# EricSteinberger/PokerRL

Measured on NVIDIA H100. Metric: CFR+ iterations/s, higher is better.
Workload: dtype f32

## Files before the change

pokerrl_b200/csrc/cfr_board.cu:

```cuda
#include <cuda_runtime.h>
#include <stdint.h>
#include <type_traits>

#include "pokerrl_b200.h"
#include "prl_common.cuh"

namespace {

constexpr int kDeck = 52;
constexpr int kBoardCards = 5;
constexpr int kLiveCards = kDeck - kBoardCards;
constexpr int kLive = kLiveCards * (kLiveCards - 1) / 2;
constexpr int kLdb = 1088;
constexpr int kRowLen = kLiveCards - 1;
constexpr int kRowPad = 48;
constexpr int kRowSeg = 12;
constexpr int kErStride = kLiveCards;
constexpr int kZeroSlot = kLive + 1;
constexpr int kRange = 1326;

constexpr int kRecBytes = kLdb * 8;
constexpr int kShBytes = kLdb * 2;
constexpr int kRowIdxBytes = kLiveCards * kRowPad * 2;
constexpr int kBlobA = kRecBytes + kShBytes;
constexpr int kBlobBytes = kBlobA + kRowIdxBytes;
static_assert(kBlobA % 16 == 0 && kRowIdxBytes % 16 == 0, "bulk copies move multiples of 16 bytes");

#ifndef PRL_BV_RED
#define PRL_BV_RED 1
#endif
#ifndef PRL_BV_P1PIPE
#define PRL_BV_P1PIPE 1
#endif
#ifndef PRL_BV_FOLDLIN
#define PRL_BV_FOLDLIN 1
#endif
#ifndef PRL_BV_ERT
#define PRL_BV_ERT 1
#endif
#ifndef PRL_BV_ROWTOTF
#define PRL_BV_ROWTOTF 1
#endif
#ifndef PRL_BV_NEWTON
#define PRL_BV_NEWTON 1
#endif
#ifndef PRL_BV_PF
#define PRL_BV_PF 1
#endif
#ifndef PRL_BV_STAMPS
#define PRL_BV_STAMPS 0
#endif
constexpr int kVP1Pipe = PRL_BV_P1PIPE;
constexpr bool kVRed = PRL_BV_RED, kVFoldLin = PRL_BV_FOLDLIN, kVErT = PRL_BV_ERT;

constexpr int kThreads = 384;
constexpr int kPerThread = 3;
constexpr int kWarps = kThreads / 32;

struct Nodes15 {
    int v[15];
};
constexpr unsigned long long pack_nodes(Nodes15 t) {
    unsigned long long r = 0;
    for (int i = 0; i < 15; ++i) r |= (unsigned long long)(t.v[i] + 1) << (4 * i);
    return r;
}
constexpr int unpack_node(unsigned long long t, int i) { return (int)((t >> (4 * i)) & 0xF) - 1; }

template <class SH>
struct ShapeOps {
    static constexpr int kind(int i) { return unpack_node(SH::kKind, i); }
    static constexpr int parent(int i) { return unpack_node(SH::kParent, i); }
    static constexpr int first_child(int i) { return unpack_node(SH::kFirstChild, i); }
    static constexpr int n_children(int i) { return unpack_node(SH::kNChildren, i); }
    static constexpr int vec_index(int i) {
        int n = 0;
        for (int k = 0; k < i; ++k) n += (kind(k) == kind(i));
        return n;
    }
// ... 28 lines not shown

struct ShapeFHP : ShapeOps<ShapeFHP> {
    static constexpr int N = 15;
    static constexpr unsigned long long kKind = pack_nodes({{1, 0, 0, 4, 1, 3, 4, 1, 3, 4, 0, 3, 4, 3, 4}});
    static constexpr unsigned long long kParent = pack_nodes({{-1, 0, 0, 1, 1, 2, 2, 2, 4, 4, 4, 7, 7, 10, 10}});
    static constexpr unsigned long long kFirstChild = pack_nodes({{1, 3, 5, -1, 8, -1, -1, 11, -1, -1, 13, -1, -1, -1, -1}});
    static constexpr unsigned long long kNChildren = pack_nodes({{2, 2, 3, 0, 3, 0, 0, 2, 0, 0, 2, 0, 0, 0, 0}});
    static constexpr int n_sd = 5, n_fold = 4;
    static constexpr int rows = 14;
    static constexpr int fold_coef(int P, int f, int v) {
        constexpr int c[2][4][5] = {{{0, 1, 0, 0, 0}, {1, 0, -1, 0, -1}, {0, 1, 0, -1, 0}, {0, 0, 0, 0, 1}},
                                    {{1, -1, 1, -1, 0}, {0, 0, 1, 0, 0}, {0, 0, 0, 1, 0}, {0, 0, 1, 0, -1}}};
        return c[P][f][v];
    }
};

struct ShapeFHPShort : ShapeOps<ShapeFHPShort> {
    static constexpr int N = 9;
    static constexpr unsigned long long kKind = pack_nodes({{1, 0, 0, 4, 1, 3, 4, 3, 4}});
    static constexpr unsigned long long kParent = pack_nodes({{-1, 0, 0, 1, 1, 2, 2, 4, 4}});
    static constexpr unsigned long long kFirstChild = pack_nodes({{1, 3, 5, -1, 7, -1, -1, -1, -1}});
    static constexpr unsigned long long kNChildren = pack_nodes({{2, 2, 2, 0, 2, 0, 0, 0, 0}});
    static constexpr int n_sd = 3, n_fold = 2;
    static constexpr int rows = 8;
    static constexpr int fold_coef(int P, int f, int v) {
        constexpr int c[2][2][3] = {{{0, 1, 0}, {1, 0, -1}}, {{1, -1, 1}, {0, 0, 1}}};
        return c[P][f][v];
    }
};

template <class SH>
constexpr bool shape_consistent() {
    return SH::count(4) == SH::n_sd && SH::count(3) == SH::n_fold && SH::rows_of_seat(0) + SH::rows_of_seat(1) == SH::rows &&
           SH::N <= 15 && SH::n_fold % 2 == 0;
}
static_assert(shape_consistent<ShapeFHP>() && shape_consistent<ShapeFHPShort>(), "shape");

template <int I, int N, class F>
__device__ __forceinline__ void static_for(F&& f) {
    if constexpr (I < N) {
        f(std::integral_constant<int, I>{});
        static_for<I + 1, N>(f);
    }
}
template <int I, int N, class F>
__device__ __forceinline__ void static_for_down(F&& f) {
    if constexpr (I < N) {
        f(std::integral_constant<int, N - 1>{});
        static_for_down<I, N - 1>(f);
    }
}

constexpr int kErVec = kLiveCards * kErStride;
template <class SH>
struct SweepSmem {
    static constexpr int kNVec = SH::n_sd + SH::n_fold;
    static constexpr int kSOff = 0;
    static constexpr int kErOff = kSOff + kNVec * kLdb * 4;
    static constexpr int kErBytes = ((SH::n_sd * kErVec * 4) + 15) & ~15;
    static constexpr int kBlobOff = kErOff + kErBytes;
    static constexpr int kRowIdxOff = kBlobOff + 2 * kBlobA;
    static constexpr int kCsOff = kRowIdxOff + kRowIdxBytes;
    static constexpr int kCsdOff = kCsOff + SH::n_fold * kRowPad * 4;
    static constexpr int kMiscOff = kCsdOff + SH::n_fold * kRowPad * 8;
    static constexpr int kMiscBytes = (SH::n_sd * 16 + SH::n_sd * 16) * 8 + 8 * 4;
    static constexpr int kRowTotOff = kMiscOff + kMiscBytes;
    static constexpr int kRowTotBytes = SH::n_sd * kRowPad * 8;
    static constexpr int kBarOff = kRowTotOff + kRowTotBytes;
    static constexpr int kSmemBytes = kBarOff + 32;
    static_assert(kBlobOff % 16 == 0 && kRowIdxOff % 16 == 0 && kCsdOff % 8 == 0 && kMiscOff % 8 == 0 && kRowTotOff % 8 == 0 &&
                      kBarOff % 8 == 0, "alignment");
    static_assert(2 * (kSmemBytes + 1024) <= 233472, "two CTAs per SM (228 KB of shared memory per H100 SM)");
    static_assert(SH::n_fold <= 8, "tf[8]");
};

struct SweepArgs {
    prl_board_game_t g;
    const float* trunk_reach_opp;
    int iter, delay;
    float m_old, m_new;
    int pair;
    float m_old_due, m_new_due;
    int src_own, src_opp;
    float rw;
    float defer_w;
    double fx_scale;
    float sc[16];
};

__device__ __forceinline__ uint32_t smem_u32(const void* p) { return (uint32_t)__cvta_generic_to_shared(p); }
__device__ __forceinline__ void mbar_init(uint64_t* bar, int count) {
    asm volatile("mbarrier.init.shared::cta.b64 [%0], %1;" ::"r"(smem_u32(bar)), "r"(count) : "memory");
}
__device__ __forceinline__ void mbar_expect_tx(uint64_t* bar, uint32_t bytes) {
    asm volatile("mbarrier.arrive.expect_tx.shared::cta.b64 _, [%0], %1;" ::"r"(smem_u32(bar)), "r"(bytes) : "memory");
}
__device__ __forceinline__ void bulk_g2s(void* dst, const void* src, uint32_t bytes, uint64_t* bar) {
    asm volatile("cp.async.bulk.shared::cluster.global.mbarrier::complete_tx::bytes [%0], [%1], %2, [%3];" ::"r"(smem_u32(dst)),
                 "l"(src), "r"(bytes), "r"(smem_u32(bar))
                 : "memory");
}
__device__ __forceinline__ void bulk_prefetch_l2(const void* src, uint32_t bytes) {
    asm volatile("cp.async.bulk.prefetch.L2.global [%0], %1;" ::"l"(src), "r"(bytes) : "memory");
}
__device__ __forceinline__ void mbar_wait(uint64_t* bar, uint32_t parity) {
    uint32_t ok;
    do {
        asm volatile(
            "{\n\t.reg .pred p;\n\tmbarrier.try_wait.parity.shared::cta.b64 p, [%1], %2;\n\tselp.u32 %0, 1, 0, p;\n\t}"
            : "=r"(ok)
            : "r"(smem_u32(bar)), "r"(parity)
            : "memory");
    } while (!ok);
}
__device__ __forceinline__ void fence_async_shared() { asm volatile("fence.proxy.async.shared::cta;" ::: "memory"); }

#if PRL_BV_STAMPS
constexpr int kStampCtas = 512, kStampUnits = 16, kStampEvery = 32, kStampSlots = 8;
__device__ long long g_stamps[kStampCtas * kStampUnits * kStampSlots];
#endif
__device__ __forceinline__ void stamp(int it, int slot) {
#if PRL_BV_STAMPS
    if (threadIdx.x == 0 && blockIdx.x < kStampCtas && it % kStampEvery == 0 && it / kStampEvery < kStampUnits) {
        long long* r = g_stamps + ((size_t)blockIdx.x * kStampUnits + it / kStampEvery) * kStampSlots;
        r[slot] = clock64();
        if (slot == 0) {
            unsigned smid;
            asm volatile("mov.u32 %0, %%smid;" : "=r"(smid));
            r[6] = smid;
            r[7] = it;
        }
    }
#endif
}

template <int A>
__device__ __forceinline__ void node_strategy(const float (&g)[A], int src, float (&s)[A]) {
    if (src == 1) {
#pragma unroll
        for (int a = 0; a < A; ++a) s[a] = g[a];
        return;
    }
    float sum = 0.0f;
#pragma unroll
    for (int a = 0; a < A; ++a) {
        s[a] = fmaxf(g[a], 0.0f);
        sum += s[a];
    }
    const bool pos = sum > 0.0f;
    const float sm = fmaxf(sum, 1e-37f);
    float inv;
    asm("rcp.approx.ftz.f32 %0, %1;" : "=f"(inv) : "f"(sm));
    if (PRL_BV_NEWTON) inv = fmaf(inv, fmaf(-sm, inv, 1.0f), inv);
    inv = pos ? inv : 0.0f;
    const float uni = pos ? 0.0f : 1.0f / (float)A;
#pragma unroll
    for (int a = 0; a < A; ++a) s[a] = fmaf(s[a], inv, uni);
}

__device__ __forceinline__ float avg_step(float m_old, float avg, float m_new, float s) {
    return __fmaf_rn(m_old, avg, __fmul_rn(m_new, s));
}

__device__ __forceinline__ float ld_stream(const float* p) { return __ldcs(p); }
__device__ __forceinline__ void st_stream(float* p, float v) { __stcs(p, v); }

template <class SH, int P, bool EVAL, bool DEFER = false, bool P1ONLY = false, bool AVG = true>
__global__ void __launch_bounds__(kThreads, 2) board_sweep_kernel(const SweepArgs a) {
    static_assert(!(EVAL && DEFER) && (!P1ONLY || DEFER) && (AVG || (!EVAL && !DEFER)), "variants");
    using M = SweepSmem<SH>;
    constexpr int NSD = SH::n_sd, NF = SH::n_fold;
    extern __shared__ __align__(128) unsigned char smem[];
    float* S = reinterpret_cast<float*>(smem + M::kSOff);
    float* Er = reinterpret_cast<float*>(smem + M::kErOff);
    float* cs = reinterpret_cast<float*>(smem + M::kCsOff);
    double* csd = reinterpret_cast<double*>(smem + M::kCsdOff);
    double* wsum = reinterpret_cast<double*>(smem + M::kMiscOff);
    double* wexc = wsum + NSD * 16;
    float* tf = reinterpret_cast<float*>(wexc + NSD * 16);
    uint64_t* bars = reinterpret_cast<uint64_t*>(smem + M::kBarOff);
    const int16_t* rowidx = reinterpret_cast<const int16_t*>(smem + M::kRowIdxOff);
    double* rowtot = reinterpret_cast<double*>(smem + M::kRowTotOff);
    constexpr bool kLin = kVFoldLin && !EVAL;

    const int tid = threadIdx.x, lane = tid & 31, warp = tid >> 5;
    const prl_board_game_t& G = a.g;
    const int nb = G.n_boards;
    constexpr int OPP = 1 - P;
    constexpr int ROWS = SH::rows;
    constexpr int OWN0 = (P == 0) ? 0 : SH::rows_of_seat(0);
    constexpr int OPP0 = (P == 0) ? SH::rows_of_seat(0) : 0;
    constexpr int NOWN = SH::rows_of_seat(P), NOPP = SH::rows_of_seat(OPP);
    constexpr size_t kBoardFloats = (size_t)ROWS * kLdb;
    const unsigned char* blob_g = reinterpret_cast<const unsigned char*>(G.tables);
    const float* tab_opp = (EVAL && a.src_opp >= 1) ? G.avg : G.regret;
    const float* tab_own = (EVAL && a.src_own >= 1) ? G.avg : G.regret;
    const int asis_opp = (EVAL && a.src_opp == 1) ? 1 : 0, asis_own = (EVAL && a.src_own == 1) ? 1 : 0;
    const bool do_avg = !EVAL && !DEFER && AVG && a.iter >= a.delay;
    const bool pair = do_avg && a.pair;
    const bool defer_now = DEFER && a.defer_w != 0.0f;
    const bool read_avg = do_avg && (pair ? a.m_old_due : a.m_old) != 0.0f;

    long long* wp = reinterpret_cast<long long*>(G.w_private) + (size_t)blockIdx.x * 2 * kRange;
    for (int h = tid; h < 2 * kRange; h += kThreads) wp[h] = 0;
    for (int v = 0; v < M::kNVec; ++v)
        for (int i = kLive + tid; i < kLdb; i += kThreads) S[v * kLdb + i] = 0.0f;
    if (tid == 0) {
        mbar_init(&bars[0], 1);
        mbar_init(&bars[1], 1);
        mbar_init(&bars[2], 1);
        fence_async_shared();
    }
    __syncthreads();
    int j = blockIdx.x;
    auto prefetch_rows = [&](int jj) {
        bulk_prefetch_l2(tab_opp + (size_t)jj * kBoardFloats + (size_t)OPP0 * kLdb, NOPP * kLdb * 4);
        bulk_prefetch_l2(tab_own + (size_t)jj * kBoardFloats + (size_t)OWN0 * kLdb, NOWN * kLdb * 4);
        if (read_avg) bulk_prefetch_l2(G.avg + (size_t)jj * kBoardFloats + (size_t)OWN0 * kLdb, NOWN * kLdb * 4);
        if (defer_now) bulk_prefetch_l2(G.avg + (size_t)jj * kBoardFloats + (size_t)OPP0 * kLdb, NOPP * kLdb * 4);
    };
    constexpr bool kPfPhase = PRL_BV_PF && !EVAL;
    auto prefetch_opp = [&](int jj) {
        bulk_prefetch_l2(tab_opp + (size_t)jj * kBoardFloats + (size_t)OPP0 * kLdb, NOPP * kLdb * 4);
        if (defer_now) bulk_prefetch_l2(G.avg + (size_t)jj * kBoardFloats + (size_t)OPP0 * kLdb, NOPP * kLdb * 4);
    };
    auto prefetch_own = [&](int jj) {
        bulk_prefetch_l2(tab_own + (size_t)jj * kBoardFloats + (size_t)OWN0 * kLdb, NOWN * kLdb * 4);
        if (read_avg) bulk_prefetch_l2(G.avg + (size_t)jj * kBoardFloats + (size_t)OWN0 * kLdb, NOWN * kLdb * 4);
    };
    if (tid == 0 && j < nb) {
        mbar_expect_tx(&bars[0], kBlobA);
        bulk_g2s(smem + M::kBlobOff, blob_g + (size_t)j * kBlobBytes, kBlobA, &bars[0]);
        if (!P1ONLY) {
            mbar_expect_tx(&bars[2], kRowIdxBytes);
            bulk_g2s(smem + M::kRowIdxOff, blob_g + (size_t)j * kBlobBytes + kBlobA, kRowIdxBytes, &bars[2]);
        }
        if constexpr (kPfPhase) prefetch_opp(j);
        else prefetch_rows(j);
    }

    constexpr int kP1Ahead = kVP1Pipe ? kVP1Pipe : kPerThread;
    float p1_g[kP1Ahead][NOPP], p1_x0[kP1Ahead];
    auto p1_load_k = [&](int jj, const int16_t* sh_jj, int k, float (&g)[NOPP], float& x0) {
        const int i = min(tid + k * kThreads, kLive - 1);
        const float* rows = tab_opp + (size_t)jj * kBoardFloats + (size_t)OPP0 * kLdb + i;
#pragma unroll
        for (int r = 0; r < NOPP; ++r) g[r] = ld_stream(rows + (size_t)r * kLdb);
        x0 = __ldg(a.trunk_reach_opp + sh_jj[i]);
    };
    auto p1_load = [&](int jj, const int16_t* sh_jj) {
#pragma unroll
        for (int k = 0; k < kP1Ahead; ++k) p1_load_k(jj, sh_jj, k, p1_g[k], p1_x0[k]);
    };

    for (int it = 0; j < nb; j += gridDim.x, ++it) {
        const int buf = it & 1;
        const unsigned char* blob = smem + M::kBlobOff + buf * kBlobA;
        const uint64_t* rec = reinterpret_cast<const uint64_t*>(blob);
        const int16_t* sh = reinterpret_cast<const int16_t*>(blob + kRecBytes);
        const int jn = j + gridDim.x;
        stamp(it, 0);
        if (tid == 0 && jn < nb) {
            mbar_expect_tx(&bars[buf ^ 1], kBlobA);
            bulk_g2s(smem + M::kBlobOff + (buf ^ 1) * kBlobA, blob_g + (size_t)jn * kBlobBytes, kBlobA, &bars[buf ^ 1]);
            if constexpr (!kPfPhase) prefetch_rows(jn);
        }
        const float prob = __ldg(G.board_prob + j);
        if (it == 0) {
            mbar_wait(&bars[buf], 0);
            p1_load(j, sh);
        }

        auto p1_hand = [&](int k, const float (&gk)[NOPP], float x0k) {
            const int i = tid + k * kThreads;
            if (i < kLive) {
                float x[SH::N];
                x[0] = x0k * prob;
                static_for<0, SH::N>([&](auto I) {
                    constexpr int n = decltype(I)::value;
                    constexpr int A = SH::n_children(n);
                    if constexpr (SH::kind(n) <= 1) {
                        constexpr int fc = SH::first_child(n);
                        if constexpr (SH::kind(n) == OPP) {
                            constexpr int r0 = SH::row_of(fc);
                            float gg[A], s[A];
#pragma unroll
                            for (int c = 0; c < A; ++c) gg[c] = gk[r0 - OPP0 + c];
                            node_strategy<A>(gg, asis_opp, s);
#pragma unroll
                            for (int c = 0; c < A; ++c) x[fc + c] = x[n] * s[c];
                            if constexpr (DEFER) {
                                if (defer_now) {
                                    float* arow = G.avg + (size_t)j * kBoardFloats + i;
#pragma unroll
                                    for (int c = 0; c < A; ++c) {
                                        float* ap = arow + (size_t)(r0 + c) * kLdb;
                                        st_stream(ap, __fadd_rn(ld_stream(ap), __fmul_rn(x[fc + c], a.defer_w)));
                                    }
                                }
                            }
                        } else {
#pragma unroll
                            for (int c = 0; c < A; ++c) x[fc + c] = x[n];
                        }
                    } else if constexpr (SH::kind(n) == 4) {
                        S[SH::vec_index(n) * kLdb + i] = x[n];
                    } else {
                        S[(NSD + SH::vec_index(n)) * kLdb + i] = x[n];
                    }
                });
            }
        };
        if constexpr (kVP1Pipe == 1) {
            float gB[NOPP], gC[NOPP], xB = 0.0f, xC = 0.0f;
            p1_load_k(j, sh, 1, gB, xB);
            p1_hand(0, p1_g[0], p1_x0[0]);
            p1_load_k(j, sh, 2, gC, xC);
            p1_hand(1, gB, xB);
            p1_hand(2, gC, xC);
        } else {
#pragma unroll
            for (int k = 0; k < kPerThread; ++k) p1_hand(k, p1_g[k], p1_x0[k]);
        }
        __syncthreads();
        stamp(it, 1);
        if (kPfPhase && tid == 0) {
            if constexpr (P1ONLY) {
                if (jn < nb) prefetch_opp(jn);
            } else {
                prefetch_own(j);
            }
        }
        if constexpr (!P1ONLY) {

        mbar_wait(&bars[2], it & 1);
        float a0[NSD], a1[NSD], a2[NSD];
        double pre[NSD];
        constexpr int kQuadThreads = kLiveCards * 4;
        constexpr int kSdSplit = (NSD + 1) / 2, kFoldSplit = NF / 2;
        if (warp < (2 * kQuadThreads + 31) / 32) {
            const int grp = (tid >= kQuadThreads) ? 1 : 0;
            const int t = tid - grp * kQuadThreads;
            const bool row_live = t < kQuadThreads;
            const int lc = row_live ? (t >> 2) : (kLiveCards - 1), q = tid & 3;
            const unsigned qmask = 0xFu << (lane & 28);
            const uint2* rp = reinterpret_cast<const uint2*>(rowidx + lc * kRowPad + q * kRowSeg);
            const uint2 w0 = rp[0], w1 = rp[1], w2 = rp[2];
            const unsigned pk[6] = {w0.x, w0.y, w1.x, w1.y, w2.x, w2.y};
            int idx[kRowSeg];
#pragma unroll
            for (int e = 0; e < kRowSeg; ++e) idx[e] = (pk[e >> 1] >> ((e & 1) * 16)) & 0xffffu;
            const int v_lo = grp ? kSdSplit : 0, v_hi = grp ? NSD : kSdSplit;
#pragma unroll 1
            for (int v = v_lo; v < v_hi; ++v) {
                const float* Sv = S + v * kLdb;
                float inc[kRowSeg];
                float run = 0.0f;
                double drun = 0.0;
#pragma unroll
                for (int e = 0; e < kRowSeg; ++e) {
                    const float xv = Sv[idx[e]];
                    inc[e] = run;
                    run += xv;
                    if constexpr (kLin && !PRL_BV_ROWTOTF) drun += (double)xv;
                }
                if constexpr (kLin) {
                    if constexpr (PRL_BV_ROWTOTF) drun = (double)run;
                    drun += __shfl_xor_sync(qmask, drun, 1, 4);
                    drun += __shfl_xor_sync(qmask, drun, 2, 4);
                    if (row_live && q == 0) rowtot[v * kRowPad + lc] = drun;
                }
                float sc = run;
                float tt = __shfl_up_sync(qmask, sc, 1, 4);
                if (q >= 1) sc += tt;
                tt = __shfl_up_sync(qmask, sc, 2, 4);
                if (q >= 2) sc += tt;
                const float half = 0.5f * __shfl_sync(qmask, sc, 3, 4);
                const float off = (sc - run) - half;
                float* row = Er + v * kErVec + (kVErT ? q * kRowSeg * kErStride + lc : lc * kErStride + q * kRowSeg);
#pragma unroll
                for (int e = 0; e < kRowSeg; ++e)
                    if (row_live && q * kRowSeg + e < kErStride) row[kVErT ? e * kErStride : e] = off + inc[e];
            }
#pragma unroll 1
            for (int f = kFoldSplit * grp; f < (kLin ? 0 : kFoldSplit * grp + kFoldSplit); ++f) {
                const float* Sv = S + (NSD + f) * kLdb;
                double run = 0.0;
#pragma unroll
                for (int e = 0; e < kRowSeg; ++e) run += (double)Sv[idx[e]];
                run += __shfl_xor_sync(qmask, run, 1, 4);
                run += __shfl_xor_sync(qmask, run, 2, 4);
                if (row_live && q == 0) csd[f * kRowPad + lc] = run;
            }
        }
        __syncwarp();
        {
            const int b0 = 3 * tid;
#pragma unroll
            for (int v = 0; v < NSD; ++v) {
                const float* Sv = S + v * kLdb;
                a0[v] = (b0 < kLive) ? Sv[b0] : 0.0f;
                a1[v] = (b0 + 1 < kLive) ? Sv[b0 + 1] : 0.0f;
                a2[v] = (b0 + 2 < kLive) ? Sv[b0 + 2] : 0.0f;
                const double loc = ((double)a0[v] + (double)a1[v]) + (double)a2[v];
                double incw = loc;
#pragma unroll
                for (int o = 1; o < 32; o <<= 1) {
                    const double tt = __shfl_up_sync(0xffffffffu, incw, o);
                    if (lane >= o) incw += tt;
                }
                pre[v] = incw - loc;
                if (lane == 31) wsum[v * 16 + warp] = incw;
            }
        }
        const float mult = __ldg(G.board_mult + j);
        const double fx = (double)mult * a.fx_scale;
        const float* own_rows = tab_own + (size_t)j * kBoardFloats + (size_t)OWN0 * kLdb;
        float* reg_rows = G.regret + (size_t)j * kBoardFloats + (size_t)OWN0 * kLdb;
        float* avg_rows = G.avg + (size_t)j * kBoardFloats + (size_t)OWN0 * kLdb;
        auto p3_pos = [&](int k) -> int { return tid + k * kThreads; };
        float gA[NOWN], aA[NOWN], gB[NOWN], aB[NOWN];
        auto p3_load = [&](int k, float (&g)[NOWN], float (&av)[NOWN]) {
            const int i = min(p3_pos(k), kLive - 1);
#pragma unroll
            for (int r = 0; r < NOWN; ++r) g[r] = ld_stream(own_rows + (size_t)r * kLdb + i);
#pragma unroll
            for (int r = 0; r < NOWN; ++r) av[r] = 0.0f;
            if (read_avg) {
#pragma unroll
                for (int r = 0; r < NOWN; ++r) av[r] = ld_stream(avg_rows + (size_t)r * kLdb + i);
            }
        };
        p3_load(0, gA, aA);
        __syncthreads();
        stamp(it, 2);
        if (tid == 0 && jn < nb) {
            mbar_expect_tx(&bars[2], kRowIdxBytes);
            bulk_g2s(smem + M::kRowIdxOff, blob_g + (size_t)jn * kBlobBytes + kBlobA, kRowIdxBytes, &bars[2]);
            if constexpr (kPfPhase) prefetch_opp(jn);
        }
        auto fold_finish = [&](auto F) {
            constexpr int f = decltype(F)::value;
            double c0 = 0.0, c1 = 0.0;
            if constexpr (kLin) {
                static_for<0, NSD>([&](auto V) {
                    constexpr int v = decltype(V)::value;
                    constexpr int cf = SH::fold_coef(P, f, v);
                    if constexpr (cf != 0) {
                        const double r0 = (lane < kLiveCards) ? rowtot[v * kRowPad + lane] : 0.0;
                        const double r1 = (lane + 32 < kLiveCards) ? rowtot[v * kRowPad + lane + 32] : 0.0;
                        c0 = (cf > 0) ? c0 + r0 : c0 - r0;
                        c1 = (cf > 0) ? c1 + r1 : c1 - r1;
                    }
                });
            } else {
                c0 = (lane < kLiveCards) ? csd[f * kRowPad + lane] : 0.0;
                c1 = (lane + 32 < kLiveCards) ? csd[f * kRowPad + lane + 32] : 0.0;
            }
            double s2 = c0 + c1;
#pragma unroll
            for (int o = 16; o > 0; o >>= 1) s2 += __shfl_xor_sync(0xffffffffu, s2, o);
            if (lane == 0) tf[f] = (float)(0.5 * s2);
            if (lane < kLiveCards) cs[f * kRowPad + lane] = (float)c0;
            if (lane + 32 < kLiveCards) cs[f * kRowPad + lane + 32] = (float)c1;
        };
        {
            auto warp_totals_scan = [&](int v) {
                const double w = (lane < kWarps) ? wsum[v * 16 + lane] : 0.0;
                double sc = w;
#pragma unroll
                for (int o = 1; o < 16; o <<= 1) {
                    const double tt = __shfl_up_sync(0xffffffffu, sc, o);
                    if (lane >= o) sc += tt;
                }
                const double total = __shfl_sync(0xffffffffu, sc, kWarps - 1);
                if (lane < kWarps) wexc[v * 16 + lane] = (sc - w) - 0.5 * total;
            };
            if (warp == 0) {
#pragma unroll
                for (int v = 0; v < NSD; ++v) warp_totals_scan(v);
            } else if (warp == 1) {
                static_for<0, NF>([&](auto F) { fold_finish(F); });
            }
            __syncthreads();
            stamp(it, 3);
            const int b0 = 3 * tid;
#pragma unroll
            for (int v = 0; v < NSD; ++v) {
                float* Sv = S + v * kLdb;
                double run = pre[v] + wexc[v * 16 + warp];
                if (b0 <= kLive) Sv[b0] = (float)run;
                run += (double)a0[v];
                if (b0 + 1 <= kLive) Sv[b0 + 1] = (float)run;
                run += (double)a1[v];
                if (b0 + 2 <= kLive) Sv[b0 + 2] = (float)run;
            }
        }
        __syncthreads();
        stamp(it, 4);

        auto p3_hand = [&](int k, const float (&gown)[NOWN], float (&av)[NOWN]) {
            const int i = p3_pos(k);
            const uint64_t w = rec[i];
            const int hand = sh[i];
            long long* wacc = wp + hand;
            long long w_ev = 0, w_br = 0;
            if constexpr (!kVRed) {
                w_ev = *wacc;
                if constexpr (EVAL) w_br = wacc[kRange];
            }
            const int gs = (int)(w & 0x7ffu), ge = (int)((w >> 11) & 0x7ffu);
            const int lc1 = (int)((w >> 22) & 0x3fu), lc2 = (int)((w >> 28) & 0x3fu);
            const int k1 = (int)((w >> 34) & 0x3fu), t1 = (int)((w >> 40) & 0x3fu), k2 = (int)((w >> 46) & 0x3fu), t2 = (int)((w >> 52) & 0x3fu);
            const int o1 = kVErT ? k1 * kErStride + lc1 : lc1 * kErStride + k1, o1e = o1 + (kVErT ? t1 * kErStride : t1);
            const int o2 = kVErT ? k2 * kErStride + lc2 : lc2 * kErStride + k2, o2e = o2 + (kVErT ? t2 * kErStride : t2);
            float e[SH::N], br[EVAL ? SH::N : 1];
            static_for<0, SH::N>([&](auto I) {
                constexpr int n = decltype(I)::value;
                if constexpr (SH::kind(n) == 4) {
                    constexpr int v = SH::vec_index(n);
                    const float* Ev = S + v * kLdb;
                    const float* Rv = Er + v * kErVec;
                    const float all = Ev[gs] + Ev[ge];
                    const float rows = (Rv[o1] + Rv[o1e]) + (Rv[o2] + Rv[o2e]);
                    e[n] = (all - rows) * a.sc[n];
                    if constexpr (EVAL) br[n] = e[n];
                } else if constexpr (SH::kind(n) == 3) {
                    constexpr int f = SH::vec_index(n);
                    const float mass = ((tf[f] - cs[f * kRowPad + lc1]) - cs[f * kRowPad + lc2]) + S[(NSD + f) * kLdb + i];
                    e[n] = mass * a.sc[n];
                    if constexpr (EVAL) br[n] = e[n];
                }
            });
            static_for_down<0, SH::N>([&](auto I) {
                constexpr int n = decltype(I)::value;
                constexpr int A = SH::n_children(n);
                if constexpr (SH::kind(n) <= 1) {
                    constexpr int fc = SH::first_child(n);
                    if constexpr (SH::kind(n) == OPP) {
                        float v = e[fc];
#pragma unroll
                        for (int c = 1; c < A; ++c) v += e[fc + c];
                        e[n] = v;
                        if constexpr (EVAL) {
                            float b = br[fc];
#pragma unroll
                            for (int c = 1; c < A; ++c) b += br[fc + c];
                            br[n] = b;
                        }
                    } else {
                        constexpr int r0 = SH::row_of(fc) - OWN0;
                        float g[A], s[A];
#pragma unroll
                        for (int c = 0; c < A; ++c) g[c] = gown[r0 + c];
                        node_strategy<A>(g, asis_own, s);
                        if (pair) {
#pragma unroll
                            for (int c = 0; c < A; ++c) av[r0 + c] = avg_step(a.m_old_due, av[r0 + c], a.m_new_due, s[c]);
                        }
                        float v = s[0] * e[fc];
#pragma unroll
                        for (int c = 1; c < A; ++c) v += s[c] * e[fc + c];
                        e[n] = v;
                        if constexpr (EVAL) {
                            float b = br[fc];
#pragma unroll
                            for (int c = 1; c < A; ++c) b = fmaxf(b, br[fc + c]);
                            br[n] = b;
                        } else {
#pragma unroll
                            for (int c = 0; c < A; ++c) {
                                if constexpr (DEFER) g[c] = __fadd_rn(__fmul_rn(a.rw, e[fc + c] - v), g[c]);
                                else g[c] = fmaxf((e[fc + c] - v) + g[c], 0.0f);
                            }
                            if constexpr (!DEFER) node_strategy<A>(g, 0, s);
#pragma unroll
                            for (int c = 0; c < A; ++c) st_stream(reg_rows + (size_t)(r0 + c) * kLdb + i, g[c]);
                            if (do_avg) {
#pragma unroll
                                for (int c = 0; c < A; ++c)
                                    st_stream(avg_rows + (size_t)(r0 + c) * kLdb + i, avg_step(a.m_old, av[r0 + c], a.m_new, s[c]));
                            }
                        }
                    }
                }
            });
            if constexpr (kVRed) {
                atomicAdd(reinterpret_cast<unsigned long long*>(wacc), (unsigned long long)__double2ll_rn((double)e[0] * fx));
                if constexpr (EVAL)
                    atomicAdd(reinterpret_cast<unsigned long long*>(wacc + kRange), (unsigned long long)__double2ll_rn((double)br[0] * fx));
            } else {
                *wacc = w_ev + __double2ll_rn((double)e[0] * fx);
                if constexpr (EVAL) wacc[kRange] = w_br + __double2ll_rn((double)br[0] * fx);
            }
        };
        p3_load(1, gB, aB);
        p3_hand(0, gA, aA);
        p3_load(2, gA, aA);
        if (p3_pos(1) < kLive) p3_hand(1, gB, aB);
        if (p3_pos(2) < kLive) p3_hand(2, gA, aA);
        }
        if (jn < nb) {
            mbar_wait(&bars[buf ^ 1], ((it + 1) >> 1) & 1);
            p1_load(jn, reinterpret_cast<const int16_t*>(smem + M::kBlobOff + (buf ^ 1) * kBlobA + kRecBytes));
        }
        __syncthreads();
        stamp(it, 5);
    }
    __syncthreads();
    unsigned long long* wt = reinterpret_cast<unsigned long long*>(G.w_total) + (EVAL ? 2 * P * kRange : 0);
    for (int h = tid; h < (EVAL ? 2 : 1) * kRange; h += kThreads) {
        const long long v = __ldcg(wp + h);
        if (v != 0) atomicAdd(wt + h, (unsigned long long)v);
    }
}

template <class SH, int P>
__global__ void __launch_bounds__(256) avg_flush_kernel(float* __restrict__ regret, float* __restrict__ avg, float m_old, float m_new) {
    constexpr size_t kBoardFloats = (size_t)SH::rows * kLdb;
    const float* reg_b = regret + (size_t)blockIdx.x * kBoardFloats;
    float* avg_b = avg + (size_t)blockIdx.x * kBoardFloats;
    for (int i = threadIdx.x; i < kLive; i += blockDim.x) {
        static_for<0, SH::N>([&](auto I) {
            constexpr int n = decltype(I)::value;
            if constexpr (SH::kind(n) == P) {
                constexpr int A = SH::n_children(n), r0 = SH::row_of(SH::first_child(n));
                float g[A], s[A];
#pragma unroll
                for (int c = 0; c < A; ++c) g[c] = ld_stream(reg_b + (size_t)(r0 + c) * kLdb + i);
                node_strategy<A>(g, 0, s);
#pragma unroll
                for (int c = 0; c < A; ++c) {
                    float* ap = avg_b + (size_t)(r0 + c) * kLdb + i;
                    st_stream(ap, avg_step(m_old, (m_old != 0.0f) ? ld_stream(ap) : 0.0f, m_new, s[c]));
                }
            }
        });
    }
}

__global__ void __launch_bounds__(256) board_tables_kernel(const int32_t* __restrict__ ranks, const uint64_t* __restrict__ board_mask,
                                                           const int8_t* __restrict__ hand_cards, int n_boards,
                                                           unsigned char* __restrict__ out) {
    __shared__ int srk[kRange];
    __shared__ short spos[kRange], sgs[kRange], sge[kRange];
    const int b = blockIdx.x;
    const uint64_t bm = board_mask[b];
    unsigned char* blob = out + (size_t)b * kBlobBytes;
    uint64_t* rec = reinterpret_cast<uint64_t*>(blob);
    int16_t* sh = reinterpret_cast<int16_t*>(blob + kRecBytes);
    int16_t* rowidx = reinterpret_cast<int16_t*>(blob + kBlobA);
    for (int h = threadIdx.x; h < kRange; h += blockDim.x) srk[h] = ranks[(size_t)b * kRange + h];
    for (int i = threadIdx.x; i < kLdb; i += blockDim.x) {
        rec[i] = 0;
        sh[i] = 0;
    }
    for (int i = threadIdx.x; i < kLiveCards * kRowPad; i += blockDim.x) rowidx[i] = (int16_t)kZeroSlot;
    __syncthreads();
    for (int h = threadIdx.x; h < kRange; h += blockDim.x) {
        const int r = srk[h];
        int lt = 0, le = 0, tb = 0;
        if (r >= 0) {
            for (int q = 0; q < kRange; ++q) {
                const int x = srk[q];
                if (x < 0) continue;
                lt += x < r;
                le += x <= r;
                tb += (x == r) && (q < h);
            }
        }
        sgs[h] = (short)(r >= 0 ? lt : -1);
        sge[h] = (short)(r >= 0 ? le : -1);
        spos[h] = (short)(r >= 0 ? lt + tb : -1);
    }
    __syncthreads();
    for (int it = threadIdx.x; it < kDeck * (kDeck - 1); it += blockDim.x) {
        const int c = it / (kDeck - 1), xr = it % (kDeck - 1);
        const int x = xr + (xr >= c);
        if (((bm >> c) | (bm >> x)) & 1ull) continue;
        const int c1 = min(c, x), c2 = max(c, x);
        const int h = c1 * (2 * kDeck - 1 - c1) / 2 + (c2 - c1 - 1);
        const int g = sgs[h], ps = spos[h];
        int lt = 0, le = 0, kpos = 0;
        for (int y = 0; y < kDeck; ++y) {
            if (y == c || ((bm >> y) & 1ull)) continue;
            const int d1 = min(c, y), d2 = max(c, y);
            const int h2 = d1 * (2 * kDeck - 1 - d1) / 2 + (d2 - d1 - 1);
            const int g2 = sgs[h2];
            lt += g2 < g;
            le += g2 <= g;
            kpos += spos[h2] < ps;
        }
        const int lc = c - __popcll(bm & ((1ull << c) - 1ull));
        rowidx[lc * kRowPad + kpos] = (int16_t)ps;
        const uint64_t fld = ((uint64_t)lc) << (c == c1 ? 22 : 28) | ((uint64_t)lt) << (c == c1 ? 34 : 46) |
                             ((uint64_t)(le - lt)) << (c == c1 ? 40 : 52);
        atomicOr(reinterpret_cast<unsigned long long*>(rec + ps), (unsigned long long)fld);
    }
    __syncthreads();
    for (int h = threadIdx.x; h < kRange; h += blockDim.x) {
        const int ps = spos[h];
        if (ps < 0) continue;
        sh[ps] = (int16_t)h;
        atomicOr(reinterpret_cast<unsigned long long*>(rec + ps),
                 (unsigned long long)((uint64_t)sgs[h] | ((uint64_t)sge[h] << 11)));
    }
}

__global__ void board_collect_kernel(const long long* __restrict__ w_total, int n_arr, const int16_t* __restrict__ sym_perm,
                                     int n_sym, double inv_scale, float* __restrict__ out, int ld) {
    const int h = blockIdx.x * blockDim.x + threadIdx.x;
    if (h >= kRange) return;
    for (int a = 0; a < n_arr; ++a) {
        long long s = 0;
        if (n_sym > 1) {
            for (int q = 0; q < n_sym; ++q) s += w_total[(size_t)a * kRange + sym_perm[(size_t)q * kRange + h]];
        } else {
            s = w_total[(size_t)a * kRange + h];
        }
        out[(size_t)a * ld + h] = (float)((double)s * inv_scale);
    }
}

__global__ void board_permute_kernel(const unsigned char* __restrict__ tables, int n_boards, int rows_per_board,
                                     const int64_t* __restrict__ row_src, const int64_t* __restrict__ row_dst, float* sorted_tab,
                                     float* natural_tab, int ld, int to_natural) {
    const int j = blockIdx.x / rows_per_board, r = blockIdx.x % rows_per_board;
    const int16_t* sh = reinterpret_cast<const int16_t*>(tables + (size_t)j * kBlobBytes + kRecBytes);
    float* srow = sorted_tab + ((size_t)row_src[2 * r] + (size_t)j * row_src[2 * r + 1]) * kLdb;
    float* nrow = natural_tab + ((size_t)row_dst[2 * r] + (size_t)j * row_dst[2 * r + 1]) * ld;
    if (to_natural) {
        for (int h = threadIdx.x; h < ld; h += blockDim.x) nrow[h] = 0.0f;
        __syncthreads();
        for (int i = threadIdx.x; i < kLive; i += blockDim.x) nrow[sh[i]] = srow[i];
    } else {
        for (int i = threadIdx.x; i < kLive; i += blockDim.x) srow[i] = nrow[sh[i]];
    }
}

__constant__ int8_t c_suit_perm[24][4] = {
    {0, 1, 2, 3}, {0, 1, 3, 2}, {0, 2, 1, 3}, {0, 2, 3, 1}, {0, 3, 1, 2}, {0, 3, 2, 1}, {1, 0, 2, 3}, {1, 0, 3, 2},
    {1, 2, 0, 3}, {1, 2, 3, 0}, {1, 3, 0, 2}, {1, 3, 2, 0}, {2, 0, 1, 3}, {2, 0, 3, 1}, {2, 1, 0, 3}, {2, 1, 3, 0},
    {2, 3, 0, 1}, {2, 3, 1, 0}, {3, 0, 1, 2}, {3, 0, 2, 1}, {3, 1, 0, 2}, {3, 1, 2, 0}, {3, 2, 0, 1}, {3, 2, 1, 0}};


__device__ __forceinline__ int hand_index(int c1, int c2) {
    return c1 * (2 * kDeck - 1 - c1) / 2 + (c2 - c1 - 1);
}

template <class SH>
__global__ void __launch_bounds__(256) policy_query_kernel(const float* __restrict__ rows, const long long* __restrict__ keys,
                                                           const int16_t* __restrict__ pos_hand, int n_cls, int iso,
                                                           const int8_t* __restrict__ boards, const int32_t* __restrict__ out_index,
                                                           unsigned long long act, int n_actions, float* __restrict__ out,
                                                           int* __restrict__ miss) {
    __shared__ short s_pos[kRange];
    __shared__ long long s_key[24];
    __shared__ int s_perm, s_cls;
    constexpr int kNDec = SH::n_dec();
    const int q = blockIdx.x, tid = threadIdx.x;
    int cards[kBoardCards];
    uint64_t bm = 0;
#pragma unroll
    for (int k = 0; k < kBoardCards; ++k) {
        cards[k] = boards[(size_t)q * kBoardCards + k];
        bm |= 1ull << cards[k];
    }
    if (tid < 24) {
        const int s = iso ? tid : 0;
        int m[kBoardCards];
#pragma unroll
        for (int k = 0; k < kBoardCards; ++k) m[k] = (cards[k] >> 2) * 4 + c_suit_perm[s][cards[k] & 3];
#pragma unroll
        for (int i = 1; i < kBoardCards; ++i)
#pragma unroll
            for (int j = i; j > 0; --j)
                if (m[j] < m[j - 1]) {
                    const int t = m[j];
                    m[j] = m[j - 1];
                    m[j - 1] = t;
                }
        long long key = 0;
#pragma unroll
        for (int k = 0; k < kBoardCards; ++k) key = key * 64 + m[k];
        s_key[tid] = key;
    }
    __syncthreads();
    if (tid == 0) {
        int best = 0;
        if (iso)
            for (int s = 1; s < 24; ++s)
                if (s_key[s] < s_key[best]) best = s;
        const long long k = s_key[best];
        int lo = 0, hi = n_cls;
        while (lo < hi) {
            const int mid = (lo + hi) >> 1;
            if (keys[mid] < k) lo = mid + 1;
            else hi = mid;
        }
        s_perm = best;
        s_cls = (lo < n_cls && keys[lo] == k) ? lo : -1;
// ... 187 lines not shown
            if (lane == 0) dred[warp] = v;
            __syncthreads();
            if (tid == 0) {
                double s = 0.0;
                for (int w = 0; w < kTrunkThreads / 32; ++w) s += dred[w];
                out_expl[p] = (float)s;
            }
        }
    }
}

template <class SH>
bool shape_matches(const prl_board_game_t* g) {
    if (g->n_local != SH::N) return false;
    for (int i = 0; i < SH::N; ++i)
        if (g->kind[i] != SH::kind(i) || g->parent[i] != SH::parent(i) || g->first_child[i] != SH::first_child(i) ||
            g->n_children[i] != SH::n_children(i))
            return false;
    return true;
}

template <class SH>
bool layout_matches(const prl_board_game_t* g) {
    for (int i = 1; i < SH::N; ++i)
        if (g->row0[i] != SH::row_of(i) || g->row_m[i] != SH::rows) return false;
    return true;
}

constexpr int kNoShape = -1000;
template <class F>
int with_shape(const prl_board_game_t* g, F&& f) {
    if (!g) return kNoShape;
    if (shape_matches<ShapeFHP>(g)) return f(ShapeFHP{});
    if (shape_matches<ShapeFHPShort>(g)) return f(ShapeFHPShort{});
    return kNoShape;
}

int default_grid() {
    static int cached[64] = {0};
    int dev = 0;
    cudaGetDevice(&dev);
    if (dev < 0 || dev >= 64) dev = 0;
    if (!cached[dev]) {
        int sms = 132;
        cudaDeviceGetAttribute(&sms, cudaDevAttrMultiProcessorCount, dev);
        cached[dev] = 2 * sms;
    }
    return cached[dev];
}

template <class SH, int P, bool EVAL, bool DEFER = false, bool P1ONLY = false, bool AVG = true>
int launch_sweep(const SweepArgs& a, int grid, cudaStream_t s) {
    auto kern = board_sweep_kernel<SH, P, EVAL, DEFER, P1ONLY, AVG>;
    constexpr int kSmemBytes = SweepSmem<SH>::kSmemBytes;
    cudaError_t e = cudaFuncSetAttribute(kern, cudaFuncAttributeMaxDynamicSharedMemorySize, kSmemBytes);
    if (e != cudaSuccess) return prl::check(e, "prl_board_sweep: shared memory opt-in");
    kern<<<grid, kThreads, kSmemBytes, s>>>(a);
    prl::count_launch();
    return 0;
}

void cfrp_weights(int iter, int delay, float* m_old, float* m_new) {
    const double cw = 0.5 * ((double)iter * (iter + 1) - (double)delay * (delay + 1));
    const double nw = (double)iter - delay + 1;
    *m_old = (iter > delay) ? (float)(cw / (cw + nw)) : 0.0f;
    *m_new = (iter > delay) ? (float)(nw / (cw + nw)) : 1.0f;
}

}

extern "C" int prl_board_layout(const prl_board_game_t* shape, int32_t* out) {
    int n_local = 0;
    if (shape) {
        n_local = with_shape(shape, [](auto sh) { return decltype(sh)::N; });
        if (n_local == kNoShape) return prl::fail("prl_board_layout: the post-deal subtree has no compiled shape");
    }
    out[0] = kLive;
    out[1] = kLdb;
    out[2] = kBlobBytes;
    out[3] = kRecBytes;
    out[4] = kBlobA;
    out[5] = kLiveCards;
    out[6] = kRowPad;
    out[7] = n_local;
    return 0;
}

extern "C" int prl_board_grid(void) { return default_grid(); }

extern "C" int prl_board_rows(const prl_board_game_t* shape, int32_t* row_of, int32_t* rows_per_board) {
    const int rc = with_shape(shape, [&](auto sh) {
        using SH = decltype(sh);
        for (int i = 0; i < 16; ++i) row_of[i] = (i >= 1 && i < SH::N) ? SH::row_of(i) : -1;
        *rows_per_board = SH::rows;
        return 0;
    });
    return rc == kNoShape ? prl::fail("prl_board_rows: the post-deal subtree has no compiled shape") : rc;
}

extern "C" int prl_board_shape_ok(const prl_board_game_t* g) {
    return with_shape(g, [](auto) { return 1; }) == 1 ? 1 : 0;
}

extern "C" int prl_board_build_tables(const int32_t* ranks, const uint64_t* board_mask, const int8_t* hand_cards, int n_boards,
                                      void* blob, prl_stream_t stream) {
    if (n_boards <= 0) return 0;
    board_tables_kernel<<<n_boards, 256, 0, (cudaStream_t)stream>>>(ranks, board_mask, hand_cards, n_boards, (unsigned char*)blob);
// ... 176 lines not shown
```

Baseline: 64.73.

## Rebuild hand-index and row-index tables in shared memory instead of bulk-loading them

In the main training sweep variant (AVG, not EVAL or DEFER), the kernel no longer copies the per-board 16-bit hand indices or the row-index table from global memory. It derives them on chip from the packed 64-bit records and a board card mask stored in the record padding. A tie-rank byte table and a live-card map are built in shared memory, with the next board's tables built by idle warps during phase 2. This cuts per-board global and L2 traffic, at the cost of extra integer work, extra shared-memory stores and more shared memory per block.

```diff
diff --git a/pokerrl_b200/csrc/cfr_board.cu b/pokerrl_b200/csrc/cfr_board.cu
--- a/pokerrl_b200/csrc/cfr_board.cu
+++ b/pokerrl_b200/csrc/cfr_board.cu
@@ -24,7 +24,34 @@
 constexpr int kRowIdxBytes = kLiveCards * kRowPad * 2;
 constexpr int kBlobA = kRecBytes + kShBytes;
 constexpr int kBlobBytes = kBlobA + kRowIdxBytes;
-static_assert(kBlobA % 16 == 0 && kRowIdxBytes % 16 == 0, "bulk copies move multiples of 16 bytes");
+static_assert(kBlobA % 16 == 0 && kRowIdxBytes % 16 == 0 && kRecBytes % 16 == 0, "bulk copies move multiples of 16 bytes");
+static_assert(kLive < kLdb, "rec[kLdb - 1] is padding: the board's 52-bit card mask");
+
+__device__ __forceinline__ int hand_index(int c1, int c2) {
+    return c1 * (2 * kDeck - 1 - c1) / 2 + (c2 - c1 - 1);
+}
+
+constexpr int kTieWin = 24, kTieRow = 2 * kTieWin;
+constexpr int kTieBytes = kLiveCards * kTieRow;
+constexpr int kNoTie = 63;
+__device__ __forceinline__ int tie_at(int c, int x) {
+    const int h = x >= kTieWin, e = x - h * kTieWin;
+    return c * kTieRow + h * kTieWin + 4 * (e % 6) + e / 6;
+}
+__device__ __forceinline__ int tie_rank(const unsigned char* tie, int c, int x, int k, int t) {
+    const int h = x >= kTieWin, e = x - h * kTieWin;
+    const int bit = 8 * (e / 6) + e % 6;
+    const uint2* w = reinterpret_cast<const uint2*>(tie + c * kTieRow + h * kTieWin);
+    const uint32_t kk = 0x01010101u * (uint32_t)k;
+    uint32_t f = 0;
+#pragma unroll
+    for (int q = 0; q < 3; ++q) {
+        const uint2 v = w[q];
+        f |= (~((v.x ^ kk) + 0x7f7f7f7fu) & 0x80808080u) >> (7 - 2 * q);
+        f |= (~((v.y ^ kk) + 0x7f7f7f7fu) & 0x80808080u) >> (6 - 2 * q);
+    }
+    return h == 0 ? __popc(f & ((1u << bit) - 1u)) : t - 1 - __popc(f >> (bit + 1));
+}
 
 #ifndef PRL_BV_RED
 #define PRL_BV_RED 1
@@ -159,15 +186,20 @@
 }
 
 constexpr int kErVec = kLiveCards * kErStride;
-template <class SH>
+template <bool EVAL, bool DEFER, bool AVG>
+constexpr bool kSweepRebuild = AVG && !EVAL && !DEFER;
+template <class SH, bool R>
 struct SweepSmem {
     static constexpr int kNVec = SH::n_sd + SH::n_fold;
     static constexpr int kSOff = 0;
     static constexpr int kErOff = kSOff + kNVec * kLdb * 4;
     static constexpr int kErBytes = ((SH::n_sd * kErVec * 4) + 15) & ~15;
+    static constexpr int kBlobBuf = R ? kRecBytes : kBlobA;
     static constexpr int kBlobOff = kErOff + kErBytes;
-    static constexpr int kRowIdxOff = kBlobOff + 2 * kBlobA;
-    static constexpr int kCsOff = kRowIdxOff + kRowIdxBytes;
+    static constexpr int kRowIdxOff = kBlobOff + 2 * kBlobBuf;
+    static constexpr int kTieOff = kRowIdxOff + kRowIdxBytes;
+    static constexpr int kLiveOff = kTieOff + (R ? kTieBytes : 0);
+    static constexpr int kCsOff = kLiveOff + (R ? 2 * kTieRow : 0);
     static constexpr int kCsdOff = kCsOff + SH::n_fold * kRowPad * 4;
     static constexpr int kMiscOff = kCsdOff + SH::n_fold * kRowPad * 8;
     static constexpr int kMiscBytes = (SH::n_sd * 16 + SH::n_sd * 16) * 8 + 8 * 4;
@@ -175,8 +207,8 @@
     static constexpr int kRowTotBytes = SH::n_sd * kRowPad * 8;
     static constexpr int kBarOff = kRowTotOff + kRowTotBytes;
     static constexpr int kSmemBytes = kBarOff + 32;
-    static_assert(kBlobOff % 16 == 0 && kRowIdxOff % 16 == 0 && kCsdOff % 8 == 0 && kMiscOff % 8 == 0 && kRowTotOff % 8 == 0 &&
-                      kBarOff % 8 == 0, "alignment");
+    static_assert(kBlobOff % 16 == 0 && kRowIdxOff % 16 == 0 && kTieOff % 8 == 0 && kCsdOff % 8 == 0 && kMiscOff % 8 == 0 &&
+                      kRowTotOff % 8 == 0 && kBarOff % 8 == 0, "alignment");
     static_assert(2 * (kSmemBytes + 1024) <= 233472, "two CTAs per SM (228 KB of shared memory per H100 SM)");
     static_assert(SH::n_fold <= 8, "tf[8]");
 };
@@ -275,7 +307,8 @@
 template <class SH, int P, bool EVAL, bool DEFER = false, bool P1ONLY = false, bool AVG = true>
 __global__ void __launch_bounds__(kThreads, 2) board_sweep_kernel(const SweepArgs a) {
     static_assert(!(EVAL && DEFER) && (!P1ONLY || DEFER) && (AVG || (!EVAL && !DEFER)), "variants");
-    using M = SweepSmem<SH>;
+    constexpr bool kRebuild = kSweepRebuild<EVAL, DEFER, AVG>;
+    using M = SweepSmem<SH, kRebuild>;
     constexpr int NSD = SH::n_sd, NF = SH::n_fold;
     extern __shared__ __align__(128) unsigned char smem[];
     float* S = reinterpret_cast<float*>(smem + M::kSOff);
@@ -286,7 +319,9 @@
     double* wexc = wsum + NSD * 16;
     float* tf = reinterpret_cast<float*>(wexc + NSD * 16);
     uint64_t* bars = reinterpret_cast<uint64_t*>(smem + M::kBarOff);
-    const int16_t* rowidx = reinterpret_cast<const int16_t*>(smem + M::kRowIdxOff);
+    int16_t* rowidx = reinterpret_cast<int16_t*>(smem + M::kRowIdxOff);
+    unsigned char* tie = smem + M::kTieOff;
+    unsigned char* live_s = smem + M::kLiveOff;
     double* rowtot = reinterpret_cast<double*>(smem + M::kRowTotOff);
     constexpr bool kLin = kVFoldLin && !EVAL;
 
@@ -312,6 +347,10 @@
     for (int h = tid; h < 2 * kRange; h += kThreads) wp[h] = 0;
     for (int v = 0; v < M::kNVec; ++v)
         for (int i = kLive + tid; i < kLdb; i += kThreads) S[v * kLdb + i] = 0.0f;
+    if constexpr (kRebuild) {
+        for (int i = tid; i < kTieBytes / 4; i += kThreads) reinterpret_cast<uint32_t*>(tie)[i] = 0x01010101u * kNoTie;
+        for (int lc = tid; lc < kLiveCards; lc += kThreads) rowidx[lc * kRowPad + kRowLen] = rowidx[lc * kRowPad + kRowLen + 1] = kZeroSlot;
+    }
     if (tid == 0) {
         mbar_init(&bars[0], 1);
         mbar_init(&bars[1], 1);
@@ -336,9 +375,9 @@
         if (read_avg) bulk_prefetch_l2(G.avg + (size_t)jj * kBoardFloats + (size_t)OWN0 * kLdb, NOWN * kLdb * 4);
     };
     if (tid == 0 && j < nb) {
-        mbar_expect_tx(&bars[0], kBlobA);
-        bulk_g2s(smem + M::kBlobOff, blob_g + (size_t)j * kBlobBytes, kBlobA, &bars[0]);
-        if (!P1ONLY) {
+        mbar_expect_tx(&bars[0], M::kBlobBuf);
+        bulk_g2s(smem + M::kBlobOff, blob_g + (size_t)j * kBlobBytes, M::kBlobBuf, &bars[0]);
+        if (!P1ONLY && !kRebuild) {
             mbar_expect_tx(&bars[2], kRowIdxBytes);
             bulk_g2s(smem + M::kRowIdxOff, blob_g + (size_t)j * kBlobBytes + kBlobA, kRowIdxBytes, &bars[2]);
         }
@@ -348,34 +387,58 @@
 
     constexpr int kP1Ahead = kVP1Pipe ? kVP1Pipe : kPerThread;
     float p1_g[kP1Ahead][NOPP], p1_x0[kP1Ahead];
-    auto p1_load_k = [&](int jj, const int16_t* sh_jj, int k, float (&g)[NOPP], float& x0) {
+    auto hand_at = [&](int b, int i) -> int {
+        const unsigned char* blob = smem + M::kBlobOff + b * M::kBlobBuf;
+        if constexpr (kRebuild) {
+            const uint64_t w = reinterpret_cast<const uint64_t*>(blob)[i];
+            const unsigned char* live = live_s + b * kTieRow;
+            return hand_index(live[(w >> 22) & 0x3f], live[(w >> 28) & 0x3f]);
+        } else {
+            return reinterpret_cast<const int16_t*>(blob + kRecBytes)[i];
+        }
+    };
+    auto unit_tables = [&](int b, int t0, int nthr) {
+        const uint64_t* r = reinterpret_cast<const uint64_t*>(smem + M::kBlobOff + b * M::kBlobBuf);
+        const uint64_t bm = r[kLdb - 1];
+        for (int c = t0; c < kDeck; c += nthr)
+            if (!((bm >> c) & 1ull)) live_s[b * kTieRow + c - __popcll(bm & ((1ull << c) - 1ull))] = (unsigned char)c;
+        for (int i = t0; i < kLive; i += nthr) {
+            const uint64_t w = r[i];
+            const int lc1 = (int)((w >> 22) & 0x3fu), lc2 = (int)((w >> 28) & 0x3fu);
+            tie[tie_at(lc1, lc2)] = (unsigned char)((w >> 34) & 0x3fu);
+            tie[tie_at(lc2, lc1)] = (unsigned char)((w >> 46) & 0x3fu);
+        }
+    };
+    auto p1_load_k = [&](int jj, int b, int k, float (&g)[NOPP], float& x0) {
         const int i = min(tid + k * kThreads, kLive - 1);
         const float* rows = tab_opp + (size_t)jj * kBoardFloats + (size_t)OPP0 * kLdb + i;
 #pragma unroll
         for (int r = 0; r < NOPP; ++r) g[r] = ld_stream(rows + (size_t)r * kLdb);
-        x0 = __ldg(a.trunk_reach_opp + sh_jj[i]);
+        x0 = __ldg(a.trunk_reach_opp + hand_at(b, i));
     };
-    auto p1_load = [&](int jj, const int16_t* sh_jj) {
-#pragma unroll
-        for (int k = 0; k < kP1Ahead; ++k) p1_load_k(jj, sh_jj, k, p1_g[k], p1_x0[k]);
+    auto p1_load = [&](int jj, int b) {
+#pragma unroll
+        for (int k = 0; k < kP1Ahead; ++k) p1_load_k(jj, b, k, p1_g[k], p1_x0[k]);
     };
 
     for (int it = 0; j < nb; j += gridDim.x, ++it) {
         const int buf = it & 1;
-        const unsigned char* blob = smem + M::kBlobOff + buf * kBlobA;
-        const uint64_t* rec = reinterpret_cast<const uint64_t*>(blob);
-        const int16_t* sh = reinterpret_cast<const int16_t*>(blob + kRecBytes);
+        const uint64_t* rec = reinterpret_cast<const uint64_t*>(smem + M::kBlobOff + buf * M::kBlobBuf);
         const int jn = j + gridDim.x;
         stamp(it, 0);
         if (tid == 0 && jn < nb) {
-            mbar_expect_tx(&bars[buf ^ 1], kBlobA);
-            bulk_g2s(smem + M::kBlobOff + (buf ^ 1) * kBlobA, blob_g + (size_t)jn * kBlobBytes, kBlobA, &bars[buf ^ 1]);
+            mbar_expect_tx(&bars[buf ^ 1], M::kBlobBuf);
+            bulk_g2s(smem + M::kBlobOff + (buf ^ 1) * M::kBlobBuf, blob_g + (size_t)jn * kBlobBytes, M::kBlobBuf, &bars[buf ^ 1]);
             if constexpr (!kPfPhase) prefetch_rows(jn);
         }
         const float prob = __ldg(G.board_prob + j);
         if (it == 0) {
             mbar_wait(&bars[buf], 0);
-            p1_load(j, sh);
+            if constexpr (kRebuild) {
+                unit_tables(buf, tid, kThreads);
+                __syncthreads();
+            }
+            p1_load(j, buf);
         }
 
         auto p1_hand = [&](int k, const float (&gk)[NOPP], float x0k) {
@@ -418,16 +481,32 @@
                 });
             }
         };
+        auto p1_rows = [&](int k) {
+            const int i = tid + k * kThreads;
+            if (kRebuild && i < kLive) {
+                const uint64_t w = rec[i];
+                const int lc1 = (int)((w >> 22) & 0x3fu), lc2 = (int)((w >> 28) & 0x3fu);
+                const int k1 = (int)((w >> 34) & 0x3fu), t1 = (int)((w >> 40) & 0x3fu), k2 = (int)((w >> 46) & 0x3fu), t2 = (int)((w >> 52) & 0x3fu);
+                rowidx[lc1 * kRowPad + k1 + (t1 > 1 ? tie_rank(tie, lc1, lc2, k1, t1) : 0)] = (int16_t)i;
+                rowidx[lc2 * kRowPad + k2 + (t2 > 1 ? tie_rank(tie, lc2, lc1, k2, t2) : 0)] = (int16_t)i;
+            }
+        };
         if constexpr (kVP1Pipe == 1) {
             float gB[NOPP], gC[NOPP], xB = 0.0f, xC = 0.0f;
-            p1_load_k(j, sh, 1, gB, xB);
+            p1_load_k(j, buf, 1, gB, xB);
             p1_hand(0, p1_g[0], p1_x0[0]);
-            p1_load_k(j, sh, 2, gC, xC);
+            p1_rows(0);
+            p1_rows(1);
+            p1_load_k(j, buf, 2, gC, xC);
             p1_hand(1, gB, xB);
+            p1_rows(2);
             p1_hand(2, gC, xC);
         } else {
 #pragma unroll
-            for (int k = 0; k < kPerThread; ++k) p1_hand(k, p1_g[k], p1_x0[k]);
+            for (int k = 0; k < kPerThread; ++k) {
+                p1_hand(k, p1_g[k], p1_x0[k]);
+                p1_rows(k);
+            }
         }
         __syncthreads();
         stamp(it, 1);
@@ -440,7 +519,7 @@
         }
         if constexpr (!P1ONLY) {
 
-        mbar_wait(&bars[2], it & 1);
+        if constexpr (!kRebuild) mbar_wait(&bars[2], it & 1);
         float a0[NSD], a1[NSD], a2[NSD];
         double pre[NSD];
         constexpr int kQuadThreads = kLiveCards * 4;
@@ -542,8 +621,10 @@
         __syncthreads();
         stamp(it, 2);
         if (tid == 0 && jn < nb) {
-            mbar_expect_tx(&bars[2], kRowIdxBytes);
-            bulk_g2s(smem + M::kRowIdxOff, blob_g + (size_t)jn * kBlobBytes + kBlobA, kRowIdxBytes, &bars[2]);
+            if constexpr (!kRebuild) {
+                mbar_expect_tx(&bars[2], kRowIdxBytes);
+                bulk_g2s(smem + M::kRowIdxOff, blob_g + (size_t)jn * kBlobBytes + kBlobA, kRowIdxBytes, &bars[2]);
+            }
             if constexpr (kPfPhase) prefetch_opp(jn);
         }
         auto fold_finish = [&](auto F) {
@@ -588,6 +669,9 @@
                 for (int v = 0; v < NSD; ++v) warp_totals_scan(v);
             } else if (warp == 1) {
                 static_for<0, NF>([&](auto F) { fold_finish(F); });
+            } else if (kRebuild && jn < nb) {
+                mbar_wait(&bars[buf ^ 1], ((it + 1) >> 1) & 1);
+                unit_tables(buf ^ 1, tid - 64, kThreads - 64);
             }
             __syncthreads();
             stamp(it, 3);
@@ -609,8 +693,7 @@
         auto p3_hand = [&](int k, const float (&gown)[NOWN], float (&av)[NOWN]) {
             const int i = p3_pos(k);
             const uint64_t w = rec[i];
-            const int hand = sh[i];
-            long long* wacc = wp + hand;
+            long long* wacc = wp + hand_at(buf, i);
             long long w_ev = 0, w_br = 0;
             if constexpr (!kVRed) {
                 w_ev = *wacc;
@@ -709,7 +792,7 @@
         }
         if (jn < nb) {
             mbar_wait(&bars[buf ^ 1], ((it + 1) >> 1) & 1);
-            p1_load(jn, reinterpret_cast<const int16_t*>(smem + M::kBlobOff + (buf ^ 1) * kBlobA + kRecBytes));
+            p1_load(jn, buf ^ 1);
         }
         __syncthreads();
         stamp(it, 5);
@@ -759,7 +842,7 @@
     int16_t* rowidx = reinterpret_cast<int16_t*>(blob + kBlobA);
     for (int h = threadIdx.x; h < kRange; h += blockDim.x) srk[h] = ranks[(size_t)b * kRange + h];
     for (int i = threadIdx.x; i < kLdb; i += blockDim.x) {
-        rec[i] = 0;
+        rec[i] = (i == kLdb - 1) ? bm : 0;
         sh[i] = 0;
     }
     for (int i = threadIdx.x; i < kLiveCards * kRowPad; i += blockDim.x) rowidx[i] = (int16_t)kZeroSlot;
@@ -849,11 +932,6 @@
     {0, 1, 2, 3}, {0, 1, 3, 2}, {0, 2, 1, 3}, {0, 2, 3, 1}, {0, 3, 1, 2}, {0, 3, 2, 1}, {1, 0, 2, 3}, {1, 0, 3, 2},
     {1, 2, 0, 3}, {1, 2, 3, 0}, {1, 3, 0, 2}, {1, 3, 2, 0}, {2, 0, 1, 3}, {2, 0, 3, 1}, {2, 1, 0, 3}, {2, 1, 3, 0},
     {2, 3, 0, 1}, {2, 3, 1, 0}, {3, 0, 1, 2}, {3, 0, 2, 1}, {3, 1, 0, 2}, {3, 1, 2, 0}, {3, 2, 0, 1}, {3, 2, 1, 0}};
-
-
-__device__ __forceinline__ int hand_index(int c1, int c2) {
-    return c1 * (2 * kDeck - 1 - c1) / 2 + (c2 - c1 - 1);
-}
 
 template <class SH>
 __global__ void __launch_bounds__(256) policy_query_kernel(const float* __restrict__ rows, const long long* __restrict__ keys,
@@ -1147,7 +1225,7 @@
 template <class SH, int P, bool EVAL, bool DEFER = false, bool P1ONLY = false, bool AVG = true>
 int launch_sweep(const SweepArgs& a, int grid, cudaStream_t s) {
     auto kern = board_sweep_kernel<SH, P, EVAL, DEFER, P1ONLY, AVG>;
-    constexpr int kSmemBytes = SweepSmem<SH>::kSmemBytes;
+    constexpr int kSmemBytes = SweepSmem<SH, kSweepRebuild<EVAL, DEFER, AVG>>::kSmemBytes;
     cudaError_t e = cudaFuncSetAttribute(kern, cudaFuncAttributeMaxDynamicSharedMemorySize, kSmemBytes);
     if (e != cudaSuccess) return prl::check(e, "prl_board_sweep: shared memory opt-in");
     kern<<<grid, kThreads, kSmemBytes, s>>>(a);
```

Result: faster. 65.84 (median of 6 runs) (+1.7%).
